# 2gunsu/monocon-pytorch

Measured on AMD Instinct MI355X. Metric: images/sec (384x1280) fwd+bwd, higher is better.
Workload: dtype f32 (f16x2); 1 GPU; train step B=32/GPU 3x384x1280 (configs[2] shape, fp32 values, mode f16x2); global_batch=32, parallelism=dp1, precision_mode=f16x2

## Files before the change

### include/monocon_hip.h

```cpp
#ifndef MONOCON_HIP_H
#define MONOCON_HIP_H

#include <stddef.h>
#include <stdint.h>

#ifdef __cplusplus
extern "C" {
#endif

typedef struct mc_handle mc_handle;

enum { MC_F32 = 0, MC_I64 = 1 };

typedef struct mc_tensor_desc {
    const char *name;
    void *ptr;
    int64_t numel;
    int32_t dtype;
} mc_tensor_desc;

enum {
    MC_PRED_CENTER_HEATMAP = 0, MC_PRED_KPT_HEATMAP, MC_PRED_WH, MC_PRED_OFFSET,
    MC_PRED_KPT_HEATMAP_OFFSET, MC_PRED_CENTER2KPT_OFFSET, MC_PRED_DIM, MC_PRED_DEPTH,
    MC_PRED_ALPHA_CLS, MC_PRED_ALPHA_OFFSET, MC_NUM_PREDS
// ... 79 lines not shown
int mc_clip_adamw_step(mc_handle *h, double lr, double beta1, double beta2, double eps,
                       double weight_decay, double max_norm, int step, float *out_norm, void *stream);

#define MC_OPT_MAX_CLASSES 16
typedef struct mc_optim_class {
    double lr, beta1, beta2, eps, weight_decay;
    int step, amsgrad, maximize;
} mc_optim_class;
int mc_optim_bind_classes(mc_handle *h, int n, float *const params[], float *const grads[],
                          float *const exp_avg[], float *const exp_avg_sq[],
                          float *const max_exp_avg_sq[], const int64_t numel[], const int cls[]);
int mc_clip_adamw_step_classes(mc_handle *h, const mc_optim_class *classes, int ncls, double max_norm,
                               double norm_type, float *out_norm, void *stream);
int mc_clip_bind(mc_handle *h, int n, float *const grads[], const int64_t numel[]);
int mc_clip_grad_norm(mc_handle *h, double max_norm, double norm_type, float *out_norm, void *stream);

int mc_op_conv(mc_handle *h, const float *const src[], const int src_channels[], int nsrc,
               int B, int Hin, int Win, const float *weight_oihw, int Cout, int ksize,
               int stride, const float *scale, const float *bias, const float *residual,
               int relu, float *out, void *stream);
int mc_op_conv_wgrad(mc_handle *h, const float *const src[], const int src_channels[], int nsrc,
                     int B, int Hin, int Win, const float *dy, int Cout, int ksize, int stride,
                     float *dw_oihw, void *stream);
int mc_op_stem(mc_handle *h, const float *img_nchw, int B, int H, int W,
               const float *weight_oihw, const float *scale, const float *bias, float *out,
               void *stream);
int mc_op_stem_dgrad(mc_handle *h, const float *dy_nhwc, const float *weight_oihw, int B, int H, int W,
                     float *dx_nchw, void *stream);
int mc_op_stem_dgrad_fused(mc_handle *h, const float *d_nhwc, const float *y_nhwc, const float *coef,
                           const float *weight_oihw, int B, int H, int W, float *dx_nchw, void *stream);
int mc_op_maxpool2(mc_handle *h, const float *in, int B, int H, int W, int C, float *out,
                   void *stream);
int mc_op_deconv4x4(mc_handle *h, const float *in, int B, int H, int W, int C,
                    const float *weight, float *out, void *stream);
int mc_op_conv_dgrad(mc_handle *h, const float *dy, const float *weight_oihw, int B, int Hin, int Win, int CinTotal,
                     int c_off, int Cs, int Cout, int ksize, int stride, int accumulate, float *dx, void *stream);
int mc_op_nchw_to_nhwc(mc_handle *h, const float *in, int B, int C, int H, int W, float *out,
                       void *stream);
int mc_op_nhwc_to_nchw(mc_handle *h, const float *in, int B, int C, int H, int W, float *out,
                       void *stream);

int mc_preprocess(mc_handle *h, const void *img_hwc, int dtype, int H, int W, const double mean[3],
                  const double std[3], int pad_h, int pad_w, float *out_chw, void *stream);

int mc_preprocess_augmented(mc_handle *h, const unsigned char *frames_hwc, const float *params, int B, int src_h, int src_w,
                            const double mean[3], const double std[3], int pad_h, int pad_w, float *out_bchw, void *stream);
// ... 43 lines not shown
```

### monocon-pytorch_amd/csrc/mc_train_api.hip

```cpp
#include "mc_internal.h"

#include <algorithm>
#include <cmath>
#include <cstdlib>
#include <cstring>
#include <vector>

static int check_targets(mc_handle *h, const mc_targets *t, const char *who) {
    if (!t) return fail(h, "%s: targets is NULL", who);
    const void *p[] = {t->center_heatmap_target, t->wh_target, t->offset_target, t->dim_target, t->alpha_cls_target,
                       t->alpha_offset_target, t->depth_target, t->center2kpt_offset_target, t->kpt_heatmap_target,
                       t->kpt_heatmap_offset_target, t->indices, t->indices_kpt, t->mask_target,
                       t->mask_center2kpt_offset, t->mask_kpt_heatmap_offset};
    for (size_t i = 0; i < sizeof(p) / sizeof(p[0]); ++i)
        if (!p[i]) return fail(h, "%s: targets field %d is NULL", who, (int)i);
    return 0;
}

extern "C" {

int mc_make_targets(mc_handle *h, const mc_labels *lab, int B, int max_objs, int pad_h, int pad_w, int fh, int fw,
                    const mc_targets *t, void *stream) {
    if (!h) return -1;
    if (!lab || !lab->gt_bboxes || !lab->gt_labels || !lab->gt_bboxes_3d || !lab->depths || !lab->gt_kpts_2d ||
// ... 113 lines not shown
    }
    HIPCHK(h, mc::launch_focal_grad(preds[0], t->center_heatmap_target, (size_t)B * 3 * HW, aux + 0, grad_losses, 0, dpreds[0], st, wrt_pred));
    HIPCHK(h, mc::launch_focal_grad(preds[1], t->kpt_heatmap_target, (size_t)B * 9 * HW, aux + 1, grad_losses, 5, dpreds[1], st, wrt_pred));
    mc::GatherLossArgs g{};
    fill_gather_args(g, preds, dpreds, t, B, max_objs, (int)HW, scratch_losses, aux + 2, grad_losses);
    g.wrt_pred = wrt_pred;
    g.partial = gather_ws(h);
    HIPCHK(h, mc::launch_gathered_losses(g, 1, st));
    return 0;
}

int mc_losses_backward(mc_handle *h, const float *const preds[MC_NUM_PREDS], const mc_targets *t, int B, int max_objs,
                       int fh, int fw, const float *grad_losses, float *const dpreds[MC_NUM_PREDS], void *stream) {
    return losses_backward_impl(h, preds, t, B, max_objs, fh, fw, grad_losses, dpreds, stream, 0);
}

int mc_losses_backward_pred(mc_handle *h, const float *const preds[MC_NUM_PREDS], const mc_targets *t, int B, int max_objs,
                            int fh, int fw, const float *grad_losses, float *const dpreds[MC_NUM_PREDS], void *stream) {
    return losses_backward_impl(h, preds, t, B, max_objs, fh, fw, grad_losses, dpreds, stream, 1);
}

int mc_op_conv_wgrad(mc_handle *h, const float *const src[], const int src_channels[], int nsrc, int B, int Hin, int Win,
                     const float *dy, int Cout, int ksize, int stride, float *dw_oihw, void *stream) {
    if (!h) return -1;
    if (!src || !src_channels || !dy || !dw_oihw || nsrc < 1 || nsrc > 4) return fail(h, "mc_op_conv_wgrad: bad argument");
    if (!((ksize == 3 && (stride == 1 || stride == 2)) || (ksize == 1 && stride == 1)))
        return fail(h, "mc_op_conv_wgrad: unsupported k=%d stride=%d", ksize, stride);
    if (Cout % 4) return fail(h, "mc_op_conv_wgrad: Cout must be a multiple of 4");
    HIPCHK(h, hipSetDevice(h->device));
    hipStream_t st = static_cast<hipStream_t>(stream);
    Tensor x[4];
    std::vector<const Tensor *> xs;
    for (int i = 0; i < nsrc; ++i) {
        if (!src[i] || src_channels[i] % 16) return fail(h, "mc_op_conv_wgrad: source %d needs C %% 16 == 0", i);
        x[i] = operand_tensor(src[i], B, Hin, Win, src_channels[i]);
        xs.push_back(&x[i]);
    }
    Tensor dyt = operand_tensor(dy, B, mc::conv_out_dim(Hin, ksize, stride), mc::conv_out_dim(Win, ksize, stride), Cout);
    ScratchBuf slots;
    if (h->prec == 3) {
        size_t n[4];
        for (int i = 0; i < nsrc; ++i) n[i] = x[i].numel();
        HIPCHK(h, op_amax_slots(slots, src, n, nsrc, dy, dyt.numel(), false, st));
        for (int i = 0; i < nsrc; ++i) x[i].amax = slots.as<unsigned>() + i * mc::AMAX_WORDS;
        dyt.amax = slots.as<unsigned>() + 4 * mc::AMAX_WORDS;
    }
    mc::WgradPlan p{};
    wgrad_args(p, xs, dyt, Cout, Cout, ksize, stride, h->prec);
    void *part = nullptr;
    HIPCHK(h, hipMalloc(&part, mc::wgrad_partial_floats(p) * sizeof(float)));
    p.a.partial = static_cast<float *>(part);
    hipError_t e = mc::launch_wgrad(p, dw_oihw, st);
    hipError_t e2 = hipStreamSynchronize(st);
    (void)hipFree(part);
    HIPCHK(h, e);
    HIPCHK(h, e2);
    return 0;
}

int mc_op_conv_dgrad(mc_handle *h, const float *dy, const float *weight_oihw, int B, int Hin, int Win, int CinTotal,
                     int c_off, int Cs, int Cout, int ksize, int stride, int accumulate, float *dx, void *stream) {
    if (!h) return -1;
    if (!dy || !weight_oihw || !dx) return fail(h, "mc_op_conv_dgrad: null argument");
    if (!((ksize == 3 && (stride == 1 || stride == 2)) || (ksize == 1 && stride == 1)))
        return fail(h, "mc_op_conv_dgrad: unsupported k=%d stride=%d", ksize, stride);
    if (Cout % 16 || Cs % 4 || c_off < 0 || c_off + Cs > CinTotal) return fail(h, "mc_op_conv_dgrad: bad channel arguments");
    if (stride == 2 && ((Hin | Win) & 1)) return fail(h, "mc_op_conv_dgrad: stride 2 needs even Hin, Win");
    HIPCHK(h, hipSetDevice(h->device));
    hipStream_t st = static_cast<hipStream_t>(stream);
    const int Ho = mc::conv_out_dim(Hin, ksize, stride), Wo = mc::conv_out_dim(Win, ksize, stride);
    const int nclass = stride == 2 ? 4 : 1;
// ... 195 lines not shown
```

### monocon-pytorch_amd/csrc/wgrad_pipe.hip

```cpp
#include <cstdlib>
#include "conv_mfma.h"
#include "train.h"

namespace mc {

typedef _Float16 h16x8 __attribute__((ext_vector_type(8)));
typedef unsigned w32x4 __attribute__((ext_vector_type(4)));
template <int V> struct WpInt { static constexpr int value = V; };

template <int KS, int WN, int WC, int WK>
struct WgPipeCfg {
    static constexpr int NB = 32 * WN, CB = 32 * WC, NW = WN * WC * WK, NT = 64 * NW;
    static constexpr int PAD = KS / 2, IH = 3 + KS, IW = 7 + KS, T = KS * KS;
    static constexpr int XROW = KS == 3 ? 32 : 16;
    static constexpr int XCH = IH * XROW + 48, DCH = 4 * 16 + 48;
    static constexpr int X_PLANE = CB * XCH, D_PLANE = NB * DCH;
    static constexpr int BUF = 2 * (X_PLANE + D_PLANE);
    static constexpr size_t LDS_BYTES = 2 * BUF;
    static_assert(LDS_BYTES <= 160 * 1024, "two tile buffers per CU");
};

__device__ __forceinline__ int wp_skew(int channel) { return ((channel >> 4) & 3) * 16; }
__device__ __forceinline__ int wp_lane_chan(int li) { return ((li & 15) >= 4 && (li & 15) < 12) ? (li ^ 16) : li; }

__device__ __forceinline__ void split_pair(float x0, float x1, float s, unsigned &hi, unsigned &lo) {
    unsigned h, l;
    asm("v_fma_mixlo_f16 %0, %1, %2, 0" : "=v"(h) : "v"(x0), "v"(s));
    asm("v_fma_mixhi_f16 %0, %1, %2, 0" : "+v"(h) : "v"(x1), "v"(s));
    asm("v_fma_mixlo_f16 %0, %1, %2, -%3 op_sel_hi:[0,0,1]" : "=v"(l) : "v"(x0), "v"(s), "v"(h));
    asm("v_fma_mixhi_f16 %0, %1, %2, -%3 op_sel:[0,0,1] op_sel_hi:[0,0,1]" : "+v"(l) : "v"(x1), "v"(s), "v"(h));
    hi = h;
    lo = l;
}

__device__ __forceinline__ void wp_barrier() { asm volatile("s_waitcnt lgkmcnt(0)\n\ts_barrier" ::: "memory"); }

template <int KS, int WN, int WC, int WK, bool LZ = false>
__global__ __launch_bounds__(64 * WN * WC * WK, WN * WC * WK == 4 ? 2 : 1) void wgrad_pipe_kernel(const WgradArgs a) {
    using Cfg = WgPipeCfg<KS, WN, WC, WK>;
    constexpr int NB = Cfg::NB, CB = Cfg::CB, NT = Cfg::NT, PAD = Cfg::PAD, IH = Cfg::IH, IW = Cfg::IW, T = Cfg::T;
    constexpr int XROW = Cfg::XROW, XCH = Cfg::XCH, DCH = Cfg::DCH, XPL = Cfg::X_PLANE, DPL = Cfg::D_PLANE, BUF = Cfg::BUF;
    extern __shared__ __attribute__((aligned(16))) unsigned char lds_raw[];

    const int tid = threadIdx.x, lane = tid & 63;
    const int wave = __builtin_amdgcn_readfirstlane(tid >> 6);
    const int wk = wave / (WN * WC), wn = (wave % (WN * WC)) / WC, wc = wave % WC;
    const int g = lane >> 5, li = lane & 31;
    const int bid = xcd_order(blockIdx.x, gridDim.x);
    const int ct = __builtin_amdgcn_readfirstlane(bid % a.c_tiles);
    const int nt = __builtin_amdgcn_readfirstlane((bid / a.c_tiles) % a.n_tiles);
    const int ksb = __builtin_amdgcn_readfirstlane(bid / (a.c_tiles * a.n_tiles));
    const int kblocks = a.ksplit / WK;
    const int n0 = nt * NB, c0 = ct * CB;
    const long long G = (long long)a.B * a.groups_per_img;
    const int g_begin = __builtin_amdgcn_readfirstlane((int)(G * ksb / kblocks));
    const int g_end = __builtin_amdgcn_readfirstlane((int)(G * (ksb + 1) / kblocks));

    f32x16 acc[T];
#pragma unroll
    for (int t = 0; t < T; ++t)
#pragma unroll
        for (int r = 0; r < 16; ++r) acc[t][r] = 0.f;

    int si = 0, cbase = 0;
    while (si + 1 < a.nsrc && c0 >= cbase + a.src[si].C) { cbase += a.src[si].C; ++si; }
    const int Cs = a.src[si].C;
    const float *xsrc = a.src[si].p;
    const int cs0 = c0 - cbase;
    const int ex = f16_scale_exp(amax_read(a.amax_x[si])), ed = f16_scale_exp(amax_read(a.amax_dy));
    const float x_scale = exp2i(ex), d_scale = exp2i(ed), omul = exp2i(-ex) * exp2i(-ed);

    constexpr int XC4 = CB / 4, XPAIRS = IW / 2, XP = IH * XPAIRS * XC4, NIX = (XP + NT - 1) / NT;
    constexpr int NC4 = NB / 4, DP = 4 * 4 * NC4, NID = (DP + NT - 1) / NT;
    static_assert(NT % XC4 == 0 && NT % NC4 == 0 && IW % 2 == 0, "static channel quad per thread");
    constexpr int DEAD = -(1 << 24);
    const int xc4 = tid % XC4, dn4 = tid % NC4;
    const bool xc_ok = cs0 + xc4 * 4 < Cs && c0 + xc4 * 4 < a.Cin;
    const bool dn_ok = n0 + dn4 * 4 + 3 < a.dy_ld;
    constexpr int KX = (NT * NIX - XP + XC4 - 1) / XC4 * XC4, KD = (NT * NID - DP + NC4 - 1) / NC4 * NC4;
    static_assert(KX <= XP && KD <= DP, "duplicate items exist");
    int x_stat[NIX], x_ix[NIX], x_dst[NIX];
#pragma unroll
    for (int i = 0; i < NIX; ++i) {
        const int e0 = tid + NT * i, e = e0 < XP ? e0 : e0 - KX, item = (e / XC4) % (IH * XPAIRS);
        const int iy = item / XPAIRS, pr = item % XPAIRS;
        const int ix = pr * 2 - PAD;
        x_ix[i] = xc_ok ? ix : DEAD;
        x_stat[i] = (((iy - PAD) * a.Win + ix) * Cs + cs0 + xc4 * 4) * 4;
        x_dst[i] = (xc4 * 4) * XCH + wp_skew(xc4 * 4) + iy * XROW + pr * 4;
    }
    int d_stat[NID], d_mx[NID], d_dst[NID];
#pragma unroll
    for (int i = 0; i < NID; ++i) {
        const int e0 = tid + NT * i, e = e0 < DP ? e0 : e0 - KD, item = (e / NC4) % 16;
        const int my = item / 4, mx = (item % 4) * 2;
        d_mx[i] = dn_ok ? mx : DEAD;
        d_stat[i] = ((my * a.Wout + mx) * a.dy_ld + n0 + dn4 * 4) * 4;
        d_dst[i] = 2 * XPL + (dn4 * 4) * DCH + wp_skew(dn4 * 4) + my * 16 + mx * 2;
    }

    f32x4 xv[2][NIX][2], dv[2][NID][2];
    const bool lz = LZ && a.src[si].la != nullptr;
    [[maybe_unused]] f32x4 *lz_tab = reinterpret_cast<f32x4 *>(lds_raw + 2 * BUF);
    if constexpr (LZ) {
        if (lz && tid < XC4) {
            f32x4 cA = {0.f, 0.f, 0.f, 0.f}, cB = cA;
            if (cs0 + tid * 4 < Cs && c0 + tid * 4 < a.Cin) {
                cA = *reinterpret_cast<const f32x4 *>(a.src[si].la + cs0 + tid * 4);
                cB = *reinterpret_cast<const f32x4 *>(a.src[si].lb + cs0 + tid * 4);
            }
#pragma unroll
            for (int j = 0; j < 4; ++j) { cA[j] *= x_scale; cB[j] *= x_scale; }
            lz_tab[tid] = cA;
            lz_tab[XC4 + tid] = cB;
        }
        __syncthreads();
    }
    [[maybe_unused]] const unsigned x_bytes = (unsigned)(a.Hin * a.Win * Cs) * 4u;
    [[maybe_unused]] unsigned okm[2] = {0u, 0u};
    auto fetch = [&](int gi, auto slot_c) {
        constexpr int slot = decltype(slot_c)::value;
        const int img = __builtin_amdgcn_readfirstlane(gi / a.groups_per_img);
        const int pp = gi - img * a.groups_per_img;
        const __amdgpu_buffer_rsrc_t r_x =
            make_rsrc(xsrc + (size_t)img * a.Hin * a.Win * Cs, (unsigned)(a.Hin * a.Win * Cs) * 4u);
        const __amdgpu_buffer_rsrc_t r_d =
            make_rsrc(a.dy + (size_t)img * a.Hout * a.Wout * a.dy_ld, (unsigned)(a.Hout * a.Wout * a.dy_ld) * 4u);
        const int prow = __builtin_amdgcn_readfirstlane(pp / a.ppr);
        const int oy = prow * 4, ox = (pp - prow * a.ppr) * 8;
        const int xb = (oy * a.Win + ox) * Cs * 4;
        const int db = (oy * a.Wout + ox) * a.dy_ld * 4;
        if constexpr (LZ) okm[slot] = 0u;
#pragma unroll
        for (int i = 0; i < NIX; ++i) {
            const int xx = ox + x_ix[i];
            const bool in0 = (unsigned)xx < (unsigned)a.Win, in1 = (unsigned)(xx + 1) < (unsigned)a.Win;
            const int vo0 = in0 ? xb + x_stat[i] : BUF_OOB, vo1 = in1 ? xb + x_stat[i] + Cs * 4 : BUF_OOB;
            xv[slot][i][0] = buf_load4(r_x, vo0, 0);
            xv[slot][i][1] = buf_load4(r_x, vo1, 0);
            if constexpr (LZ) okm[slot] |= (((unsigned)vo0 < x_bytes ? 1u : 0u) | ((unsigned)vo1 < x_bytes ? 2u : 0u)) << (2 * i);
        }
#pragma unroll
        for (int i = 0; i < NID; ++i) {
            const int xx = ox + d_mx[i];
            const bool in0 = (unsigned)xx < (unsigned)a.Wout, in1 = (unsigned)(xx + 1) < (unsigned)a.Wout;
            dv[slot][i][0] = buf_load4(r_d, in0 ? db + d_stat[i] : BUF_OOB, 0);
            dv[slot][i][1] = buf_load4(r_d, in1 ? db + d_stat[i] + a.dy_ld * 4 : BUF_OOB, 0);
        }
    };
    auto put = [&](unsigned char *dst, int plane, const f32x4 v0, const f32x4 v1, int chan_stride, float scale) {
#pragma unroll
        for (int j = 0; j < 4; ++j) {
            unsigned hi, lo;
            split_pair(v0[j], v1[j], scale, hi, lo);
            *reinterpret_cast<unsigned *>(dst + j * chan_stride) = hi;
            *reinterpret_cast<unsigned *>(dst + plane + j * chan_stride) = lo;
        }
    };
    auto store_x = [&](unsigned char *buf, auto slot_c, int i) {
        constexpr int slot = decltype(slot_c)::value;
// ... 1 lines not shown
            if (lz) {
                const float cap0 = ((okm[slot] >> (2 * i)) & 1u) ? __builtin_inff() : 0.f;
                const float cap1 = ((okm[slot] >> (2 * i + 1)) & 1u) ? __builtin_inff() : 0.f;
                const f32x4 lzA = lz_tab[xc4], lzB = lz_tab[XC4 + xc4];
                f32x4 t0, t1;
#pragma unroll
                for (int j = 0; j < 4; ++j) {
                    t0[j] = lazy_act(xv[slot][i][0][j], lzA[j], lzB[j], cap0);
                    t1[j] = lazy_act(xv[slot][i][1][j], lzA[j], lzB[j], cap1);
                }
                put(buf + x_dst[i], XPL, t0, t1, XCH, 1.f);
                return;
            }
        }
        put(buf + x_dst[i], XPL, xv[slot][i][0], xv[slot][i][1], XCH, x_scale);
    };
    auto store_d = [&](unsigned char *buf, auto slot_c, int i) {
        constexpr int slot = decltype(slot_c)::value;
        put(buf + d_dst[i], DPL, dv[slot][i][0], dv[slot][i][1], DCH, d_scale);
    };

    const int lc = wp_lane_chan(li);
    const int a_off = 2 * XPL + (wn * 32 + lc) * DCH + wp_skew(wn * 32 + lc) + g * 16;
    const int b_off = (wc * 32 + lc) * XCH + wp_skew(wc * 32 + lc) + g * XROW;

    auto half = [&](const unsigned char *buf, int q, auto &&mid) {
        h16x8 av[2];
#pragma unroll
        for (int z = 0; z < 2; ++z) av[z] = *reinterpret_cast<const h16x8 *>(buf + a_off + z * DPL + (2 * q) * 16);
#pragma unroll
        for (int r = 0; r < KS; ++r) {
            const unsigned char *row = buf + b_off + (2 * q + r) * XROW;
            w32x4 b0[2], b1[2], b2[2];
#pragma unroll
            for (int z = 0; z < 2; ++z) {
                const w32x4 lo = *reinterpret_cast<const w32x4 *>(row + z * XPL);
                b0[z] = lo;
                if (KS == 3) {
                    w32x4 hi4 = *reinterpret_cast<const w32x4 *>(row + z * XPL + 16);
                    asm volatile("" : "+v"(hi4));
                    const unsigned hi = hi4[0];
                    b1[z][0] = __builtin_amdgcn_alignbit(lo[1], lo[0], 16);
                    b1[z][1] = __builtin_amdgcn_alignbit(lo[2], lo[1], 16);
                    b1[z][2] = __builtin_amdgcn_alignbit(lo[3], lo[2], 16);
                    b1[z][3] = __builtin_amdgcn_alignbit(hi, lo[3], 16);
                    b2[z][0] = lo[1]; b2[z][1] = lo[2]; b2[z][2] = lo[3]; b2[z][3] = hi;
                }
            }
            constexpr int PA[3] = {1, 0, 0}, PX[3] = {0, 1, 0};
#pragma unroll
            for (int pp = 0; pp < 3; ++pp) {
                const int za = PA[pp], zx = PX[pp];
                if (KS == 1) {
                    acc[0] = __builtin_amdgcn_mfma_f32_32x32x16_f16(av[za], __builtin_bit_cast(h16x8, b0[zx]), acc[0], 0, 0, 0);
                } else {
                    acc[r * 3 + 0] = __builtin_amdgcn_mfma_f32_32x32x16_f16(av[za], __builtin_bit_cast(h16x8, b0[zx]), acc[r * 3 + 0], 0, 0, 0);
                    acc[r * 3 + 1] = __builtin_amdgcn_mfma_f32_32x32x16_f16(av[za], __builtin_bit_cast(h16x8, b1[zx]), acc[r * 3 + 1], 0, 0, 0);
                    acc[r * 3 + 2] = __builtin_amdgcn_mfma_f32_32x32x16_f16(av[za], __builtin_bit_cast(h16x8, b2[zx]), acc[r * 3 + 2], 0, 0, 0);
                }
            }
            if (r == 0) mid();
        }
    };

    auto iteration = [&](int gi, auto sc, auto sn) {
        unsigned char *cur = lds_raw + decltype(sc)::value * BUF, *nxt = lds_raw + decltype(sn)::value * BUF;
        auto fetch_next = [&] { fetch(min(gi + 2, g_end - 1), sc); };
        auto stage_next = [&] {
#pragma unroll
            for (int i = 0; i < NIX; ++i) store_x(nxt, sn, i);
#pragma unroll
            for (int i = 0; i < NID; ++i) store_d(nxt, sn, i);
        };
        if constexpr (WK == 2) {
            half(cur, wk, [&] { fetch_next(); stage_next(); });
        } else {
            half(cur, 0, fetch_next);
            half(cur, 1, stage_next);
        }
        wp_barrier();
    };

    if (g_begin < g_end) {
        fetch(g_begin, WpInt<0>{});
        fetch(min(g_begin + 1, g_end - 1), WpInt<1>{});
#pragma unroll
        for (int i = 0; i < NIX; ++i) store_x(lds_raw, WpInt<0>{}, i);
#pragma unroll
        for (int i = 0; i < NID; ++i) store_d(lds_raw, WpInt<0>{}, i);
        wp_barrier();
    }
    for (int gi = g_begin; gi < g_end; gi += 2) {
        iteration(gi, WpInt<0>{}, WpInt<1>{});
        if (gi + 1 < g_end) iteration(gi + 1, WpInt<1>{}, WpInt<0>{});
    }

    const int slice = ksb * WK + wk;
    const int c = c0 + wc * 32 + lc;
    if (c < a.Cin && c - cbase < Cs) {
#pragma unroll
        for (int t = 0; t < T; ++t)
#pragma unroll
            for (int r = 0; r < 16; ++r) {
                const int n = n0 + wn * 32 + wp_lane_chan((r & 3) + 8 * (r >> 2) + 4 * g);
                if (n < a.Cout) a.partial[(((size_t)slice * T + t) * a.Cout + n) * a.Cin + c] = acc[t][r] * omul;
            }
    }
}

template <int KS, int WN, int WC, int WK, bool LZ = false>
static hipError_t launch_wp(const WgradArgs &a, hipStream_t st) {
    using Cfg = WgPipeCfg<KS, WN, WC, WK>;
    constexpr size_t lds_bytes = Cfg::LDS_BYTES + (LZ ? 2 * (Cfg::CB / 4) * 16 : 0);
    return launch_dyn_lds<wgrad_pipe_kernel<KS, WN, WC, WK, LZ>>(lds_bytes, dim3((a.ksplit / WK) * a.n_tiles * a.c_tiles), dim3(Cfg::NT), st, a);
}

int wgrad_pipe_tile(const WgradArgs &a, int ks, int stride) {
    const char *en = std::getenv("MONOCON_HIP_WGRAD_PIPE");
    const int enabled = en ? std::atoi(en) : 1;
    if (!enabled || a.prec != 3 || stride != 1 || ks != 3) return 0;
    if (a.Wout != a.Win || a.Hout != a.Hin || a.dy_ld % 4 || !a.amax_dy) return 0;
    for (int i = 0; i < a.nsrc; ++i)
        if (!a.amax_x[i] || a.src[i].C % 4) return 0;
    auto src_mult = [&](int m) {
        for (int i = 0; i < a.nsrc; ++i)
            if (a.nsrc > 1 && a.src[i].C % m) return false;
        return true;
    };
    if (enabled == 1) return (a.Cout % 64 == 0 && a.Cin % 64 == 0 && src_mult(64)) ? 4 : 0;
    if (a.Cout >= 128 && a.Cout % 64 == 0 && a.Cin % 64 == 0 && src_mult(64)) return 1;
    if (a.Cout == 64 && a.Cin % 128 == 0 && src_mult(128)) return 2;
    if (enabled >= 3 && a.Cout == 64 && a.Cin % 64 == 0 && src_mult(64)) return 3;
    return 0;
}
hipError_t launch_wgrad_pipe(const WgradPlan &p, hipStream_t st) {
    switch (p.a.pipe) {
    case 1: return launch_wp<3, 4, 2, 1>(p.a, st);
    case 2: return launch_wp<3, 2, 4, 1>(p.a, st);
    case 3: return launch_wp<3, 2, 2, 2>(p.a, st);
    case 4: return wgrad_any_lazy(p.a) ? launch_wp<3, 2, 2, 1, true>(p.a, st) : launch_wp<3, 2, 2, 1>(p.a, st);
    default: return hipErrorInvalidValue;
    }
}

}
```

### monocon-pytorch_amd/csrc/wgrad_plan.hip

```cpp
#include <algorithm>
#include <cstdlib>
#include "conv_mfma.h"
#include "train.h"

namespace mc {

static int env_int(const char *name, int unset) { const char *e = std::getenv(name); return e ? std::atoi(e) : unset; }

void wgrad_plan(WgradPlan &p) {
    WgradArgs &a = p.a;
    const int ks = p.ks, stride = p.stride;
    a.pipe = p.WN = p.WC = 0; p.ok = true;
    if (wgrad_is_small(a, ks, stride)) {
        a.kernel = wgrad_thin_ok(a, ks, stride) ? WG_THIN16 : WG_SMALL;
        p.lazy_ok = a.prec == 3 && (a.kernel == WG_THIN16 || (stride == 2 && a.Cout == 32));
        const int rows = a.B * a.Hout;
        a.ksplit = std::min(rows / 4 > 0 ? rows / 4 : 1, 1024);
        a.n_tiles = a.c_tiles = 1; a.ppr = a.ppi = a.groups_per_img = 0;
    } else {
        int budget, WK = 1;
        if (const int tile = wgrad_pipe_tile(a, ks, stride)) {
            a.kernel = WG_PIPE; a.pipe = tile; a.pb = 1;
            p.WN = tile == 1 ? 4 : 2; p.WC = tile == 2 ? 4 : 2; WK = tile == 3 ? 2 : 1;
            p.lazy_ok = tile == 4;
            budget = env_int("MONOCON_HIP_WGRAD_PIPE_BLOCKS", 256);
        } else {
            wgrad_shape(a, &p.WN, &p.WC);
            const bool b16 = a.prec >= 1 && wgrad_bf16_ok(a, ks, stride), src_ok = wgrad_sources_ok(a);
            a.kernel = b16 ? WG_SPLIT : WG_FP32;
            a.pb = (b16 && a.prec >= 2) ? 1 : 2;
            p.lazy_ok = a.prec == 3 && b16 && src_ok;
            p.ok = src_ok && (b16 || (ks == 3 && (stride == 1 || stride == 2)) || (ks == 1 && stride == 1));
            budget = env_int("MONOCON_HIP_WGRAD_BLOCKS", 512) * 4 / (p.WN * p.WC);
        }
        a.n_tiles = (a.Cout + 32 * p.WN - 1) / (32 * p.WN);
        a.c_tiles = (a.Cin + 32 * p.WC - 1) / (32 * p.WC);
        wgrad_set_patches(a, a.pb);
        const long long G = (long long)a.B * a.groups_per_img;
        a.ksplit = (int)std::min<long long>(std::max(budget / (a.n_tiles * a.c_tiles), 1), G) * WK;
    }
    if (wgrad_any_lazy(a) && !p.lazy_ok) p.ok = false;
    p.partial_floats = (size_t)a.ksplit * ks * ks * a.Cout * a.Cin;
}

hipError_t launch_wgrad(const WgradPlan &p, float *dw_oihw, hipStream_t st) {
    const WgradArgs &a = p.a;
    if (!p.ok) return hipErrorInvalidValue;
    prof_last = {2, 2.0 * a.B * a.Hout * a.Wout * (double)a.Cout * a.Cin * p.ks * p.ks,
                 4.0 * ((double)a.B * a.Hin * a.Win * a.Cin + (double)a.B * a.Hout * a.Wout * a.Cout + (double)p.ks * p.ks * a.Cin * a.Cout)};
    hipError_t e = hipErrorInvalidValue;
    switch (a.kernel) {
    case WG_FP32: e = launch_wgrad_fp32(p, st); break;
    case WG_SPLIT: e = launch_wgrad_bf16(p, st); break;
    case WG_PIPE: e = launch_wgrad_pipe(p, st); break;
    case WG_SMALL: e = launch_wgrad_small(p, st); break;
    case WG_THIN16: e = launch_wgrad_thin(p, st); break;
    }
    if (e != hipSuccess) return e;
    return launch_splitk_reduce(a.partial, a.ksplit, p.ks * p.ks, a.Cout, a.Cin, dw_oihw, st);
}
// ... 3 lines not shown
```

### monocon-pytorch_amd/hipmonocon/engine.py

```python
import ctypes as C

import numpy as np
import torch

from . import lib as _lib
from . import netspec

PRED_KEYS = tuple(k for k, _ in netspec.PRED_KEYS)
PRED_CH = tuple(c for _, c in netspec.PRED_KEYS)


def _stream():
    return C.c_void_p(torch.cuda.current_stream().cuda_stream)


def _ptr(t):
    return C.c_void_p(t.data_ptr()) if t is not None else C.c_void_p(0)


def _need_cuda(t, what):
    if not (torch.is_tensor(t) and t.is_cuda):
        raise _lib.MonoconHipError("%s must be a CUDA(HIP) tensor; libmonocon_hip has no CPU path" % what)
    if not t.is_contiguous():
        raise _lib.MonoconHipError("%s must be contiguous" % what)
# ... 441 lines not shown
        Wo = (W + 2 * (k // 2) - k) // stride + 1
        out = torch.empty((B, Ho, Wo, Cout), dtype=torch.float32, device=srcs[0].device)
        sp = (C.c_void_p * len(srcs))(*[s.data_ptr() for s in srcs])
        sc = (C.c_int * len(srcs))(*[s.shape[3] for s in srcs])
        with torch.cuda.device(out.device):
            rc = self.lib.mc_op_conv(self.h, sp, sc, len(srcs), B, H, W, _ptr(_need_cuda(weight, "weight")), Cout, k,
                                     stride, _ptr(scale), _ptr(bias), _ptr(residual), int(relu), _ptr(out), _stream())
        _lib.check(self.h, rc, "mc_op_conv")
        return out

    def op_conv_dgrad(self, dy, weight, in_hw, c_off=0, cs=None, stride=1, accumulate_into=None):
        _need_cuda(dy, "dy"); _need_cuda(weight, "weight")
        B, Ho, Wo, Cout = dy.shape
        _, cin_total, k, _ = weight.shape
        cs = cin_total - c_off if cs is None else cs
        Hin, Win = in_hw
        out = accumulate_into if accumulate_into is not None else torch.empty((B, Hin, Win, cs), dtype=torch.float32, device=dy.device)
        with torch.cuda.device(dy.device):
            rc = self.lib.mc_op_conv_dgrad(self.h, _ptr(dy), _ptr(weight), B, Hin, Win, cin_total, c_off, cs, Cout, k, stride,
                                           int(accumulate_into is not None), _ptr(out), _stream())
        _lib.check(self.h, rc, "mc_op_conv_dgrad")
        return out

    def op_conv_wgrad(self, srcs, dy, ksize, stride=1):
        B, H, W, _ = srcs[0].shape
        Cout = dy.shape[3]
        cin = sum(s.shape[3] for s in srcs)
        dw = torch.empty((Cout, cin, ksize, ksize), dtype=torch.float32, device=dy.device)
        sp = (C.c_void_p * len(srcs))(*[_need_cuda(s, "src").data_ptr() for s in srcs])
        sc = (C.c_int * len(srcs))(*[s.shape[3] for s in srcs])
        with torch.cuda.device(dy.device):
            rc = self.lib.mc_op_conv_wgrad(self.h, sp, sc, len(srcs), B, H, W, _ptr(_need_cuda(dy, "dy")), Cout, ksize,
                                           stride, _ptr(dw), _stream())
        _lib.check(self.h, rc, "mc_op_conv_wgrad")
        return dw

    def op_stem(self, img, weight, scale, bias):
        B, _, H, W = img.shape
        out = torch.empty((B, H, W, 16), dtype=torch.float32, device=img.device)
        with torch.cuda.device(out.device):
            rc = self.lib.mc_op_stem(self.h, _ptr(_need_cuda(img, "img")), B, H, W, _ptr(weight), _ptr(scale),
                                     _ptr(bias), _ptr(out), _stream())
        _lib.check(self.h, rc, "mc_op_stem")
        return out

    def op_maxpool2(self, x):
        B, H, W, Cc = x.shape
        out = torch.empty((B, H // 2, W // 2, Cc), dtype=torch.float32, device=x.device)
        with torch.cuda.device(out.device):
            rc = self.lib.mc_op_maxpool2(self.h, _ptr(_need_cuda(x, "x")), B, H, W, Cc, _ptr(out), _stream())
        _lib.check(self.h, rc, "mc_op_maxpool2")
        return out

    def op_deconv4x4(self, x, weight):
        B, H, W, Cc = x.shape
        out = torch.empty((B, 2 * H, 2 * W, Cc), dtype=torch.float32, device=x.device)
# ... 32 lines not shown
```

### monocon-pytorch_amd/hipmonocon/lib.py

```python
import ctypes as C
import os

_HERE = os.path.dirname(os.path.abspath(__file__))
LIB_PATH = os.path.join(_HERE, "libmonocon_hip.so")

MC_F32, MC_I64 = 0, 1
NUM_PREDS = 10

EXPORTS = (
    "mc_create", "mc_destroy", "mc_last_error", "mc_version", "mc_bind_params", "mc_pack_params",
    "mc_forward_infer", "mc_backbone_forward", "mc_neck_forward", "mc_head_forward", "mc_decode", "mc_make_targets", "mc_losses", "mc_losses_backward", "mc_losses_backward_pred", "mc_forward_train", "mc_backward", "mc_backward_pred_grads", "mc_backward_image_grad", "mc_train_generation", "mc_head_forward_train", "mc_head_backward", "mc_head_backward_pred_grads", "mc_train_debug_node", "mc_infer_debug_node", "mc_optim_bind", "mc_clip_adamw_step", "mc_optim_bind_classes", "mc_clip_adamw_step_classes", "mc_clip_bind", "mc_clip_grad_norm", "mc_op_conv", "mc_op_conv_wgrad", "mc_op_conv_dgrad", "mc_op_stem", "mc_op_stem_dgrad", "mc_op_stem_dgrad_fused", "mc_op_maxpool2", "mc_op_deconv4x4",
    "mc_op_nchw_to_nhwc", "mc_op_nhwc_to_nchw", "mc_workspace_bytes", "mc_query_workspace", "mc_forward_cost",
    "mc_preprocess", "mc_preprocess_augmented", "mc_profile_forward", "mc_profile_train", "mc_set_precision", "mc_set_local_maximum_kernel", "mc_set_conv_cfg", "mc_bench_conv", "mc_bench_mfma_peak",
    "mc_comm_unique_id", "mc_comm_init", "mc_comm_destroy", "mc_comm_set_overlap", "mc_comm_info", "mc_comm_exposed_ms", "mc_allreduce_grads",
    "mc_build_train_plan", "mc_tune_export", "mc_tune_import",
    "mc_rotate_iou_eval", "mc_box3d_overlap", "mc_kitti_image_overlap", "mc_kitti_statistics_part",
    "mc_kitti_format", "mc_nms3d",
)


class TensorDesc(C.Structure):
    _fields_ = [("name", C.c_char_p), ("ptr", C.c_void_p), ("numel", C.c_int64), ("dtype", C.c_int32)]


class Labels(C.Structure):
    _fields_ = [(n, C.c_void_p) for n in ("gt_bboxes", "gt_labels", "gt_bboxes_3d", "depths", "gt_kpts_2d",
                                          "gt_kpts_valid_mask", "mask")]


TARGET_FIELDS = ("center_heatmap_target", "wh_target", "offset_target", "dim_target", "alpha_cls_target",
                 "alpha_offset_target", "depth_target", "center2kpt_offset_target", "kpt_heatmap_target",
                 "kpt_heatmap_offset_target", "indices", "indices_kpt", "mask_target", "mask_center2kpt_offset",
                 "mask_kpt_heatmap_offset")


class Targets(C.Structure):
    _fields_ = [(n, C.c_void_p) for n in TARGET_FIELDS]

# ... 41 lines not shown
    lib.mc_losses.argtypes = [vp, C.POINTER(vp), C.POINTER(Targets), i, i, i, i, vp, vp]
    lib.mc_losses_backward.argtypes = [vp, C.POINTER(vp), C.POINTER(Targets), i, i, i, i, vp, C.POINTER(vp), vp]
    lib.mc_losses_backward_pred.argtypes = lib.mc_losses_backward.argtypes
    lib.mc_forward_train.argtypes = [vp, vp, C.POINTER(Labels), i, i, i, i, C.POINTER(vp), vp, vp]
    lib.mc_backward.argtypes = [vp, vp, vp]
    lib.mc_backward_pred_grads.argtypes = [vp, vp, C.POINTER(vp), vp]
    lib.mc_backward_image_grad.argtypes = [vp, vp, C.POINTER(vp), vp, vp]
    lib.mc_head_forward_train.argtypes = [vp, vp, C.POINTER(Labels), i, i, i, i, C.POINTER(vp), vp, vp]
    lib.mc_head_backward.argtypes = [vp, vp, vp, vp]
    lib.mc_head_backward_pred_grads.argtypes = [vp, vp, C.POINTER(vp), vp, vp]
    lib.mc_train_generation.argtypes = [vp, C.POINTER(C.c_ulonglong)]
    lib.mc_train_debug_node.argtypes = [vp, i, i, vp, C.POINTER(i), vp]
    lib.mc_infer_debug_node.argtypes = [vp, i, i, vp, C.POINTER(i), vp]
    d = C.c_double
    lib.mc_optim_bind.argtypes = [vp, i, C.POINTER(vp), C.POINTER(vp), C.POINTER(vp), C.POINTER(vp), C.POINTER(C.c_int64)]
    lib.mc_clip_adamw_step.argtypes = [vp, d, d, d, d, d, d, i, vp, vp]
    lib.mc_optim_bind_classes.argtypes = [vp, i, C.POINTER(vp), C.POINTER(vp), C.POINTER(vp), C.POINTER(vp), C.POINTER(vp),
                                          C.POINTER(C.c_int64), C.POINTER(i)]
    lib.mc_clip_adamw_step_classes.argtypes = [vp, C.POINTER(OptimClass), i, d, d, vp, vp]
    lib.mc_clip_bind.argtypes = [vp, i, C.POINTER(vp), C.POINTER(C.c_int64)]
    lib.mc_clip_grad_norm.argtypes = [vp, d, d, vp, vp]
    lib.mc_op_conv.argtypes = [vp, C.POINTER(vp), C.POINTER(i), i, i, i, i, vp, i, i, i, vp, vp, vp, i, vp, vp]
    lib.mc_op_conv_wgrad.argtypes = [vp, C.POINTER(vp), C.POINTER(i), i, i, i, i, vp, i, i, i, vp, vp]
    lib.mc_op_stem.argtypes = [vp, vp, i, i, i, vp, vp, vp, vp, vp]
    lib.mc_op_stem_dgrad.argtypes = [vp, vp, vp, i, i, i, vp, vp]
    lib.mc_op_stem_dgrad_fused.argtypes = [vp, vp, vp, vp, vp, i, i, i, vp, vp]
    lib.mc_op_maxpool2.argtypes = [vp, vp, i, i, i, i, vp, vp]
    lib.mc_op_deconv4x4.argtypes = [vp, vp, i, i, i, i, vp, vp, vp]
    lib.mc_op_nchw_to_nhwc.argtypes = [vp, vp, i, i, i, i, vp, vp]
    lib.mc_op_nhwc_to_nchw.argtypes = [vp, vp, i, i, i, i, vp, vp]
    lib.mc_workspace_bytes.argtypes = [vp]
    lib.mc_query_workspace.argtypes = [vp, i, i, i, i, C.POINTER(C.c_size_t)]
    lib.mc_workspace_bytes.restype = C.c_size_t
    lib.mc_forward_cost.argtypes = [vp, i, i, i, C.POINTER(C.c_double), C.POINTER(C.c_double)]
    lib.mc_profile_forward.argtypes = [vp, i, fp, C.POINTER(i), vp]
    lib.mc_bench_mfma_peak.argtypes = [vp, i, i, fp]
    lib.mc_profile_train.argtypes = [vp, i, C.POINTER(C.c_double), C.POINTER(C.c_double), C.POINTER(C.c_double), C.POINTER(i), vp]
    lib.mc_preprocess.argtypes = [vp, vp, i, i, i, C.POINTER(C.c_double), C.POINTER(C.c_double), i, i, vp, vp]
    lib.mc_preprocess_augmented.argtypes = [vp, vp, vp, i, i, i, C.POINTER(C.c_double), C.POINTER(C.c_double), i, i, vp, vp]
    lib.mc_op_conv_dgrad.argtypes = [vp, vp, vp, i, i, i, i, i, i, i, i, i, i, vp, vp]
    lib.mc_comm_unique_id.argtypes = [vp, vp]
    lib.mc_comm_init.argtypes = [vp, i, i, vp]
    lib.mc_comm_destroy.argtypes = [vp]
    lib.mc_comm_set_overlap.argtypes = [vp, i]
    lib.mc_comm_info.argtypes = [vp, C.POINTER(i), C.POINTER(i), C.POINTER(i), C.POINTER(i), C.POINTER(C.c_ulonglong), C.c_char_p, i]
    lib.mc_comm_exposed_ms.argtypes = [vp, fp]
# ... 29 lines not shown
```

Before: 682.8 images/sec.

## Extend pipelined f16 weight-gradient kernel to stride-2 3x3 convolutions

Adds a stride-2 variant of the software-pipelined MFMA weight-gradient kernel, with two output rows per group, a deinterleaved even/odd input row layout in LDS and adjusted shift/alignbit selection. Stride-2 3x3 wgrad in f16x2 mode now routes to this kernel (tile 5, 4x1 warp layout) when Cout%128 and Cin%32 allow, instead of the generic path, and the tile can also run with lazy BN-ReLU sources. It also adds a standalone lazy wgrad API entry and a numerics digest script. The new layout and indexing risk correctness issues and a different occupancy and k-split balance.

Result: no change. 685.1 images/sec (median of 6 runs) (+0.3%).

```diff
diff --git a/include/monocon_hip.h b/include/monocon_hip.h
--- a/include/monocon_hip.h
+++ b/include/monocon_hip.h
@@ -125,6 +125,9 @@
 int mc_op_conv_wgrad(mc_handle *h, const float *const src[], const int src_channels[], int nsrc,
                      int B, int Hin, int Win, const float *dy, int Cout, int ksize, int stride,
                      float *dw_oihw, void *stream);
+int mc_op_conv_wgrad_lazy(mc_handle *h, const float *const src[], const int src_channels[], const float *const la[],
+                          const float *const lb[], const float zmax[], int nsrc, int B, int Hin, int Win, const float *dy,
+                          int Cout, int ksize, int stride, float *dw_oihw, void *stream);
 int mc_op_stem(mc_handle *h, const float *img_nchw, int B, int H, int W,
                const float *weight_oihw, const float *scale, const float *bias, float *out,
                void *stream);
diff --git a/monocon-pytorch_amd/csrc/mc_train_api.hip b/monocon-pytorch_amd/csrc/mc_train_api.hip
--- a/monocon-pytorch_amd/csrc/mc_train_api.hip
+++ b/monocon-pytorch_amd/csrc/mc_train_api.hip
@@ -159,8 +159,16 @@
 
 int mc_op_conv_wgrad(mc_handle *h, const float *const src[], const int src_channels[], int nsrc, int B, int Hin, int Win,
                      const float *dy, int Cout, int ksize, int stride, float *dw_oihw, void *stream) {
+    return mc_op_conv_wgrad_lazy(h, src, src_channels, nullptr, nullptr, nullptr, nsrc, B, Hin, Win, dy, Cout, ksize, stride, dw_oihw,
+                                 stream);
+}
+
+int mc_op_conv_wgrad_lazy(mc_handle *h, const float *const src[], const int src_channels[], const float *const la[],
+                          const float *const lb[], const float zmax[], int nsrc, int B, int Hin, int Win, const float *dy,
+                          int Cout, int ksize, int stride, float *dw_oihw, void *stream) {
     if (!h) return -1;
     if (!src || !src_channels || !dy || !dw_oihw || nsrc < 1 || nsrc > 4) return fail(h, "mc_op_conv_wgrad: bad argument");
+    if (la && (!lb || !zmax || h->prec != 3)) return fail(h, "mc_op_conv_wgrad: lazy sources need lb, zmax and precision mode 3");
     if (!((ksize == 3 && (stride == 1 || stride == 2)) || (ksize == 1 && stride == 1)))
         return fail(h, "mc_op_conv_wgrad: unsupported k=%d stride=%d", ksize, stride);
     if (Cout % 4) return fail(h, "mc_op_conv_wgrad: Cout must be a multiple of 4");
@@ -181,9 +189,19 @@
         HIPCHK(h, op_amax_slots(slots, src, n, nsrc, dy, dyt.numel(), false, st));
         for (int i = 0; i < nsrc; ++i) x[i].amax = slots.as<unsigned>() + i * mc::AMAX_WORDS;
         dyt.amax = slots.as<unsigned>() + 4 * mc::AMAX_WORDS;
+        for (int i = 0; la && i < nsrc; ++i) {
+            if (!la[i]) continue;
+            if (!lb[i] || !(zmax[i] >= 0.f)) return fail(h, "mc_op_conv_wgrad: lazy source %d needs lb and zmax >= 0", i);
+            x[i].la = la[i]; x[i].lb = lb[i];
+            HIPCHK(h, hipMemsetAsync(x[i].amax, 0, mc::AMAX_WORDS * sizeof(unsigned), st));
+            HIPCHK(h, hipStreamSynchronize(st));
+            HIPCHK(h, hipMemcpy(x[i].amax, &zmax[i], sizeof(float), hipMemcpyHostToDevice));
+        }
     }
     mc::WgradPlan p{};
     wgrad_args(p, xs, dyt, Cout, Cout, ksize, stride, h->prec);
+    if (mc::wgrad_any_lazy(p.a) && !mc::wgrad_lazy_capable(p))
+        return fail(h, "mc_op_conv_wgrad: the kernel of this shape cannot form a lazy source");
     void *part = nullptr;
     HIPCHK(h, hipMalloc(&part, mc::wgrad_partial_floats(p) * sizeof(float)));
     p.a.partial = static_cast<float *>(part);
diff --git a/monocon-pytorch_amd/csrc/wgrad_pipe.hip b/monocon-pytorch_amd/csrc/wgrad_pipe.hip
--- a/monocon-pytorch_amd/csrc/wgrad_pipe.hip
+++ b/monocon-pytorch_amd/csrc/wgrad_pipe.hip
@@ -8,12 +8,14 @@
 typedef unsigned w32x4 __attribute__((ext_vector_type(4)));
 template <int V> struct WpInt { static constexpr int value = V; };
 
-template <int KS, int WN, int WC, int WK>
+template <int KS, int WN, int WC, int WK, int S = 1>
 struct WgPipeCfg {
+    static_assert(S == 1 || (S == 2 && KS == 3 && WK == 1), "stride 2: 3x3, one half per group");
     static constexpr int NB = 32 * WN, CB = 32 * WC, NW = WN * WC * WK, NT = 64 * NW;
-    static constexpr int PAD = KS / 2, IH = 3 + KS, IW = 7 + KS, T = KS * KS;
-    static constexpr int XROW = KS == 3 ? 32 : 16;
-    static constexpr int XCH = IH * XROW + 48, DCH = 4 * 16 + 48;
+    static constexpr int GR = S == 2 ? 2 : 4;
+    static constexpr int PAD = KS / 2, IH = S == 2 ? 2 * GR + 1 : 3 + KS, IW = S == 2 ? 18 : 7 + KS, T = KS * KS;
+    static constexpr int XROW = S == 2 ? 48 : (KS == 3 ? 32 : 16);
+    static constexpr int XCH = IH * XROW + (S == 2 ? 64 : 48), DCH = GR * 16 + 48;
     static constexpr int X_PLANE = CB * XCH, D_PLANE = NB * DCH;
     static constexpr int BUF = 2 * (X_PLANE + D_PLANE);
     static constexpr size_t LDS_BYTES = 2 * BUF;
@@ -35,10 +37,10 @@
 
 __device__ __forceinline__ void wp_barrier() { asm volatile("s_waitcnt lgkmcnt(0)\n\ts_barrier" ::: "memory"); }
 
-template <int KS, int WN, int WC, int WK, bool LZ = false>
+template <int KS, int WN, int WC, int WK, bool LZ = false, int S = 1>
 __global__ __launch_bounds__(64 * WN * WC * WK, WN * WC * WK == 4 ? 2 : 1) void wgrad_pipe_kernel(const WgradArgs a) {
-    using Cfg = WgPipeCfg<KS, WN, WC, WK>;
-    constexpr int NB = Cfg::NB, CB = Cfg::CB, NT = Cfg::NT, PAD = Cfg::PAD, IH = Cfg::IH, IW = Cfg::IW, T = Cfg::T;
+    using Cfg = WgPipeCfg<KS, WN, WC, WK, S>;
+    constexpr int NB = Cfg::NB, CB = Cfg::CB, NT = Cfg::NT, PAD = Cfg::PAD, IH = Cfg::IH, IW = Cfg::IW, T = Cfg::T, GR = Cfg::GR;
     constexpr int XROW = Cfg::XROW, XCH = Cfg::XCH, DCH = Cfg::DCH, XPL = Cfg::X_PLANE, DPL = Cfg::D_PLANE, BUF = Cfg::BUF;
     extern __shared__ __attribute__((aligned(16))) unsigned char lds_raw[];
 
@@ -71,7 +73,7 @@
     const float x_scale = exp2i(ex), d_scale = exp2i(ed), omul = exp2i(-ex) * exp2i(-ed);
 
     constexpr int XC4 = CB / 4, XPAIRS = IW / 2, XP = IH * XPAIRS * XC4, NIX = (XP + NT - 1) / NT;
-    constexpr int NC4 = NB / 4, DP = 4 * 4 * NC4, NID = (DP + NT - 1) / NT;
+    constexpr int NC4 = NB / 4, DP = GR * 4 * NC4, NID = (DP + NT - 1) / NT;
     static_assert(NT % XC4 == 0 && NT % NC4 == 0 && IW % 2 == 0, "static channel quad per thread");
     constexpr int DEAD = -(1 << 24);
     const int xc4 = tid % XC4, dn4 = tid % NC4;
@@ -84,15 +86,15 @@
     for (int i = 0; i < NIX; ++i) {
         const int e0 = tid + NT * i, e = e0 < XP ? e0 : e0 - KX, item = (e / XC4) % (IH * XPAIRS);
         const int iy = item / XPAIRS, pr = item % XPAIRS;
-        const int ix = pr * 2 - PAD;
+        const int ix = (S == 2 ? (pr < 5 ? 4 * pr : 4 * (pr - 5) + 1) : pr * 2) - PAD;
         x_ix[i] = xc_ok ? ix : DEAD;
         x_stat[i] = (((iy - PAD) * a.Win + ix) * Cs + cs0 + xc4 * 4) * 4;
-        x_dst[i] = (xc4 * 4) * XCH + wp_skew(xc4 * 4) + iy * XROW + pr * 4;
+        x_dst[i] = (xc4 * 4) * XCH + wp_skew(xc4 * 4) + iy * XROW + (S == 2 && pr >= 5 ? 32 + (pr - 5) * 4 : pr * 4);
     }
     int d_stat[NID], d_mx[NID], d_dst[NID];
 #pragma unroll
     for (int i = 0; i < NID; ++i) {
-        const int e0 = tid + NT * i, e = e0 < DP ? e0 : e0 - KD, item = (e / NC4) % 16;
+        const int e0 = tid + NT * i, e = e0 < DP ? e0 : e0 - KD, item = (e / NC4) % (GR * 4);
         const int my = item / 4, mx = (item % 4) * 2;
         d_mx[i] = dn_ok ? mx : DEAD;
         d_stat[i] = ((my * a.Wout + mx) * a.dy_ld + n0 + dn4 * 4) * 4;
@@ -127,15 +129,15 @@
         const __amdgpu_buffer_rsrc_t r_d =
             make_rsrc(a.dy + (size_t)img * a.Hout * a.Wout * a.dy_ld, (unsigned)(a.Hout * a.Wout * a.dy_ld) * 4u);
         const int prow = __builtin_amdgcn_readfirstlane(pp / a.ppr);
-        const int oy = prow * 4, ox = (pp - prow * a.ppr) * 8;
-        const int xb = (oy * a.Win + ox) * Cs * 4;
+        const int oy = prow * GR, ox = (pp - prow * a.ppr) * 8;
+        const int xb = (oy * a.Win + ox) * S * Cs * 4;
         const int db = (oy * a.Wout + ox) * a.dy_ld * 4;
         if constexpr (LZ) okm[slot] = 0u;
 #pragma unroll
         for (int i = 0; i < NIX; ++i) {
-            const int xx = ox + x_ix[i];
-            const bool in0 = (unsigned)xx < (unsigned)a.Win, in1 = (unsigned)(xx + 1) < (unsigned)a.Win;
-            const int vo0 = in0 ? xb + x_stat[i] : BUF_OOB, vo1 = in1 ? xb + x_stat[i] + Cs * 4 : BUF_OOB;
+            const int xx = ox * S + x_ix[i];
+            const bool in0 = (unsigned)xx < (unsigned)a.Win, in1 = (unsigned)(xx + S) < (unsigned)a.Win;
+            const int vo0 = in0 ? xb + x_stat[i] : BUF_OOB, vo1 = in1 ? xb + x_stat[i] + S * Cs * 4 : BUF_OOB;
             xv[slot][i][0] = buf_load4(r_x, vo0, 0);
             xv[slot][i][1] = buf_load4(r_x, vo1, 0);
             if constexpr (LZ) okm[slot] |= (((unsigned)vo0 < x_bytes ? 1u : 0u) | ((unsigned)vo1 < x_bytes ? 2u : 0u)) << (2 * i);
@@ -183,7 +185,7 @@
 
     const int lc = wp_lane_chan(li);
     const int a_off = 2 * XPL + (wn * 32 + lc) * DCH + wp_skew(wn * 32 + lc) + g * 16;
-    const int b_off = (wc * 32 + lc) * XCH + wp_skew(wc * 32 + lc) + g * XROW;
+    const int b_off = (wc * 32 + lc) * XCH + wp_skew(wc * 32 + lc) + g * S * XROW;
 
     auto half = [&](const unsigned char *buf, int q, auto &&mid) {
         h16x8 av[2];
@@ -191,7 +193,7 @@
         for (int z = 0; z < 2; ++z) av[z] = *reinterpret_cast<const h16x8 *>(buf + a_off + z * DPL + (2 * q) * 16);
 #pragma unroll
         for (int r = 0; r < KS; ++r) {
-            const unsigned char *row = buf + b_off + (2 * q + r) * XROW;
+            const unsigned char *row = buf + b_off + (2 * q * S + r) * XROW;
             w32x4 b0[2], b1[2], b2[2];
 #pragma unroll
             for (int z = 0; z < 2; ++z) {
@@ -201,11 +203,18 @@
                     w32x4 hi4 = *reinterpret_cast<const w32x4 *>(row + z * XPL + 16);
                     asm volatile("" : "+v"(hi4));
                     const unsigned hi = hi4[0];
-                    b1[z][0] = __builtin_amdgcn_alignbit(lo[1], lo[0], 16);
-                    b1[z][1] = __builtin_amdgcn_alignbit(lo[2], lo[1], 16);
-                    b1[z][2] = __builtin_amdgcn_alignbit(lo[3], lo[2], 16);
-                    b1[z][3] = __builtin_amdgcn_alignbit(hi, lo[3], 16);
-                    b2[z][0] = lo[1]; b2[z][1] = lo[2]; b2[z][2] = lo[3]; b2[z][3] = hi;
+                    w32x4 sh;
+                    sh[0] = __builtin_amdgcn_alignbit(lo[1], lo[0], 16);
+                    sh[1] = __builtin_amdgcn_alignbit(lo[2], lo[1], 16);
+                    sh[2] = __builtin_amdgcn_alignbit(lo[3], lo[2], 16);
+                    sh[3] = __builtin_amdgcn_alignbit(hi, lo[3], 16);
+                    if (S == 2) {
+                        b1[z] = *reinterpret_cast<const w32x4 *>(row + z * XPL + 32);
+                        b2[z] = sh;
+                    } else {
+                        b1[z] = sh;
+                        b2[z][0] = lo[1]; b2[z][1] = lo[2]; b2[z][2] = lo[3]; b2[z][3] = hi;
+                    }
                 }
             }
             constexpr int PA[3] = {1, 0, 0}, PX[3] = {0, 1, 0};
@@ -233,7 +242,9 @@
 #pragma unroll
             for (int i = 0; i < NID; ++i) store_d(nxt, sn, i);
         };
-        if constexpr (WK == 2) {
+        if constexpr (GR == 2) {
+            half(cur, 0, [&] { fetch_next(); stage_next(); });
+        } else if constexpr (WK == 2) {
             half(cur, wk, [&] { fetch_next(); stage_next(); });
         } else {
             half(cur, 0, fetch_next);
@@ -269,18 +280,18 @@
     }
 }
 
-template <int KS, int WN, int WC, int WK, bool LZ = false>
+template <int KS, int WN, int WC, int WK, bool LZ = false, int S = 1>
 static hipError_t launch_wp(const WgradArgs &a, hipStream_t st) {
-    using Cfg = WgPipeCfg<KS, WN, WC, WK>;
+    using Cfg = WgPipeCfg<KS, WN, WC, WK, S>;
     constexpr size_t lds_bytes = Cfg::LDS_BYTES + (LZ ? 2 * (Cfg::CB / 4) * 16 : 0);
-    return launch_dyn_lds<wgrad_pipe_kernel<KS, WN, WC, WK, LZ>>(lds_bytes, dim3((a.ksplit / WK) * a.n_tiles * a.c_tiles), dim3(Cfg::NT), st, a);
+    return launch_dyn_lds<wgrad_pipe_kernel<KS, WN, WC, WK, LZ, S>>(lds_bytes, dim3((a.ksplit / WK) * a.n_tiles * a.c_tiles), dim3(Cfg::NT), st, a);
 }
 
 int wgrad_pipe_tile(const WgradArgs &a, int ks, int stride) {
     const char *en = std::getenv("MONOCON_HIP_WGRAD_PIPE");
     const int enabled = en ? std::atoi(en) : 1;
-    if (!enabled || a.prec != 3 || stride != 1 || ks != 3) return 0;
-    if (a.Wout != a.Win || a.Hout != a.Hin || a.dy_ld % 4 || !a.amax_dy) return 0;
+    if (!enabled || a.prec != 3 || (stride != 1 && stride != 2) || ks != 3) return 0;
+    if (a.Wout * stride != a.Win || a.Hout * stride != a.Hin || a.dy_ld % 4 || !a.amax_dy) return 0;
     for (int i = 0; i < a.nsrc; ++i)
         if (!a.amax_x[i] || a.src[i].C % 4) return 0;
     auto src_mult = [&](int m) {
@@ -288,6 +299,11 @@
             if (a.nsrc > 1 && a.src[i].C % m) return false;
         return true;
     };
+    if (stride == 2) {
+        const char *e2 = std::getenv("MONOCON_HIP_WGRAD_PIPE_S2");
+        if (e2 && !std::atoi(e2)) return 0;
+        return (a.Cout % 128 == 0 && a.Cin % 32 == 0 && src_mult(32)) ? 5 : 0;
+    }
     if (enabled == 1) return (a.Cout % 64 == 0 && a.Cin % 64 == 0 && src_mult(64)) ? 4 : 0;
     if (a.Cout >= 128 && a.Cout % 64 == 0 && a.Cin % 64 == 0 && src_mult(64)) return 1;
     if (a.Cout == 64 && a.Cin % 128 == 0 && src_mult(128)) return 2;
@@ -300,6 +316,7 @@
     case 2: return launch_wp<3, 2, 4, 1>(p.a, st);
     case 3: return launch_wp<3, 2, 2, 2>(p.a, st);
     case 4: return wgrad_any_lazy(p.a) ? launch_wp<3, 2, 2, 1, true>(p.a, st) : launch_wp<3, 2, 2, 1>(p.a, st);
+    case 5: return wgrad_any_lazy(p.a) ? launch_wp<3, 4, 1, 1, true, 2>(p.a, st) : launch_wp<3, 4, 1, 1, false, 2>(p.a, st);
     default: return hipErrorInvalidValue;
     }
 }
diff --git a/monocon-pytorch_amd/csrc/wgrad_plan.hip b/monocon-pytorch_amd/csrc/wgrad_plan.hip
--- a/monocon-pytorch_amd/csrc/wgrad_plan.hip
+++ b/monocon-pytorch_amd/csrc/wgrad_plan.hip
@@ -21,8 +21,8 @@
         int budget, WK = 1;
         if (const int tile = wgrad_pipe_tile(a, ks, stride)) {
             a.kernel = WG_PIPE; a.pipe = tile; a.pb = 1;
-            p.WN = tile == 1 ? 4 : 2; p.WC = tile == 2 ? 4 : 2; WK = tile == 3 ? 2 : 1;
-            p.lazy_ok = tile == 4;
+            p.WN = (tile == 1 || tile == 5) ? 4 : 2; p.WC = tile == 2 ? 4 : (tile == 5 ? 1 : 2); WK = tile == 3 ? 2 : 1;
+            p.lazy_ok = tile >= 4;
             budget = env_int("MONOCON_HIP_WGRAD_PIPE_BLOCKS", 256);
         } else {
             wgrad_shape(a, &p.WN, &p.WC);
@@ -36,6 +36,7 @@
         a.n_tiles = (a.Cout + 32 * p.WN - 1) / (32 * p.WN);
         a.c_tiles = (a.Cin + 32 * p.WC - 1) / (32 * p.WC);
         wgrad_set_patches(a, a.pb);
+        if (a.pipe == 5) a.groups_per_img = a.ppr * ((a.Hout + 1) / 2);
         const long long G = (long long)a.B * a.groups_per_img;
         a.ksplit = (int)std::min<long long>(std::max(budget / (a.n_tiles * a.c_tiles), 1), G) * WK;
     }
diff --git a/monocon-pytorch_amd/hipmonocon/engine.py b/monocon-pytorch_amd/hipmonocon/engine.py
--- a/monocon-pytorch_amd/hipmonocon/engine.py
+++ b/monocon-pytorch_amd/hipmonocon/engine.py
@@ -487,7 +487,7 @@
         _lib.check(self.h, rc, "mc_op_conv_dgrad")
         return out
 
-    def op_conv_wgrad(self, srcs, dy, ksize, stride=1):
+    def op_conv_wgrad(self, srcs, dy, ksize, stride=1, lazy=None):
         B, H, W, _ = srcs[0].shape
         Cout = dy.shape[3]
         cin = sum(s.shape[3] for s in srcs)
@@ -495,8 +495,16 @@
         sp = (C.c_void_p * len(srcs))(*[_need_cuda(s, "src").data_ptr() for s in srcs])
         sc = (C.c_int * len(srcs))(*[s.shape[3] for s in srcs])
         with torch.cuda.device(dy.device):
-            rc = self.lib.mc_op_conv_wgrad(self.h, sp, sc, len(srcs), B, H, W, _ptr(_need_cuda(dy, "dy")), Cout, ksize,
-                                           stride, _ptr(dw), _stream())
+            if lazy is None:
+                rc = self.lib.mc_op_conv_wgrad(self.h, sp, sc, len(srcs), B, H, W, _ptr(_need_cuda(dy, "dy")), Cout, ksize,
+                                               stride, _ptr(dw), _stream())
+            else:
+                lz = [None if l is None else (_need_cuda(l[0], "la"), _need_cuda(l[1], "lb")) for l in lazy]
+                zmax = [0.0 if l is None else float(torch.relu(s * l[0] + l[1]).max()) for s, l in zip(srcs, lz)]
+                pa = (C.c_void_p * len(srcs))(*[None if l is None else l[0].data_ptr() for l in lz])
+                pb = (C.c_void_p * len(srcs))(*[None if l is None else l[1].data_ptr() for l in lz])
+                rc = self.lib.mc_op_conv_wgrad_lazy(self.h, sp, sc, pa, pb, (C.c_float * len(srcs))(*zmax), len(srcs), B, H, W,
+                                                    _ptr(_need_cuda(dy, "dy")), Cout, ksize, stride, _ptr(dw), _stream())
         _lib.check(self.h, rc, "mc_op_conv_wgrad")
         return dw
 
diff --git a/monocon-pytorch_amd/hipmonocon/lib.py b/monocon-pytorch_amd/hipmonocon/lib.py
--- a/monocon-pytorch_amd/hipmonocon/lib.py
+++ b/monocon-pytorch_amd/hipmonocon/lib.py
@@ -13,7 +13,7 @@
     "mc_op_nchw_to_nhwc", "mc_op_nhwc_to_nchw", "mc_workspace_bytes", "mc_query_workspace", "mc_forward_cost",
     "mc_preprocess", "mc_preprocess_augmented", "mc_profile_forward", "mc_profile_train", "mc_set_precision", "mc_set_local_maximum_kernel", "mc_set_conv_cfg", "mc_bench_conv", "mc_bench_mfma_peak",
     "mc_comm_unique_id", "mc_comm_init", "mc_comm_destroy", "mc_comm_set_overlap", "mc_comm_info", "mc_comm_exposed_ms", "mc_allreduce_grads",
-    "mc_build_train_plan", "mc_tune_export", "mc_tune_import",
+    "mc_build_train_plan", "mc_tune_export", "mc_tune_import", "mc_op_conv_wgrad_lazy",
     "mc_rotate_iou_eval", "mc_box3d_overlap", "mc_kitti_image_overlap", "mc_kitti_statistics_part",
     "mc_kitti_format", "mc_nms3d",
 )
@@ -101,6 +101,8 @@
     lib.mc_clip_grad_norm.argtypes = [vp, d, d, vp, vp]
     lib.mc_op_conv.argtypes = [vp, C.POINTER(vp), C.POINTER(i), i, i, i, i, vp, i, i, i, vp, vp, vp, i, vp, vp]
     lib.mc_op_conv_wgrad.argtypes = [vp, C.POINTER(vp), C.POINTER(i), i, i, i, i, vp, i, i, i, vp, vp]
+    lib.mc_op_conv_wgrad_lazy.argtypes = [vp, C.POINTER(vp), C.POINTER(i), C.POINTER(vp), C.POINTER(vp), C.POINTER(C.c_float),
+                                          i, i, i, i, vp, i, i, i, vp, vp]
     lib.mc_op_stem.argtypes = [vp, vp, i, i, i, vp, vp, vp, vp, vp]
     lib.mc_op_stem_dgrad.argtypes = [vp, vp, vp, i, i, i, vp, vp]
     lib.mc_op_stem_dgrad_fused.argtypes = [vp, vp, vp, vp, vp, i, i, i, vp, vp]
diff --git a/scratch/one_step_digest.py b/scratch/one_step_digest.py
--- /dev/null
+++ b/scratch/one_step_digest.py
@@ -0,0 +1,28 @@
+import hashlib, json, os, sys
+import numpy as np
+import torch
+REPO = os.path.dirname(os.path.dirname(os.path.abspath(__file__)))
+for p in (os.path.join(REPO, "monocon-pytorch_amd"), REPO):
+    sys.path.insert(0, p)
+from hipmonocon import synth
+from model import MonoConDetector
+stats = np.load(os.path.join(REPO, "tests", "golden", "bn_calib_seed7.npz"))
+def dg(t): return hashlib.sha256(t.detach().float().cpu().contiguous().numpy().tobytes()).hexdigest()[:16]
+out = {}
+for (B, H, W) in ((4, 128, 224), (2, 384, 1280)):
+    sd = synth.make_state_dict(7, bn_stats={k: stats[k] for k in stats.files})
+    m = MonoConDetector(34, pretrained_backbone=False)
+    m.load_state_dict(sd, strict=True)
+    m = m.cuda().train().set_precision("f16x2")
+    b = synth.make_batch(500, B, H, W)
+    bt = {"img": b["img"].cuda().contiguous(), "label": {k: v.cuda().contiguous() for k, v in b["label"].items()},
+          "img_metas": {"pad_shape": [(H, W)] * B}}
+    preds, loss = m(bt)
+    sum(loss.values()).backward()
+    torch.cuda.synchronize()
+    out["%dx%dx%d" % (B, H, W)] = {"loss": {k: dg(v) for k, v in sorted(loss.items())}, "pred": {k: dg(v) for k, v in sorted(preds.items())},
+                                   "grad": {n: dg(p.grad) for n, p in m.named_parameters() if p.grad is not None},
+                                   "gradval": {n: p.grad.detach().cpu().double() for n, p in m.named_parameters() if p.grad is not None and "level" in n and n.endswith("tree1.conv1.weight")}}
+vals = {s: o.pop("gradval") for s, o in out.items()}
+torch.save(vals, sys.argv[1] + ".pt")
+json.dump(out, open(sys.argv[1] + ".json", "w"), sort_keys=True)
diff --git a/scratch/one_step_digest_cmp.py b/scratch/one_step_digest_cmp.py
--- /dev/null
+++ b/scratch/one_step_digest_cmp.py
@@ -0,0 +1,10 @@
+import json, sys, torch
+a, b = json.load(open(sys.argv[1] + ".json")), json.load(open(sys.argv[2] + ".json"))
+va, vb = torch.load(sys.argv[1] + ".pt"), torch.load(sys.argv[2] + ".pt")
+for s in a:
+    print(s, "losses equal:", a[s]["loss"] == b[s]["loss"], " prediction maps equal:", a[s]["pred"] == b[s]["pred"], "(%d maps)" % len(a[s]["pred"]))
+    diff = [n for n in a[s]["grad"] if a[s]["grad"][n] != b[s]["grad"][n]]
+    print(s, "parameter gradients: %d tensors, differing: %s" % (len(a[s]["grad"]), diff))
+    for n in diff:
+        if n in va[s]:
+            print("   %s  max |a-b| / max |a| = %.3e" % (n, float((va[s][n] - vb[s][n]).abs().max() / va[s][n].abs().max())))
```
